# snap-research/InstantRestore

Hardware: AMD Instinct MI355X
Metric: restored images/sec @512px, 4 refs, single-step; 1/2/4/8 MI355X (higher is better)
Workload: dtype bf16

## Files before the change

instantrestore_amd/csrc/linear_tiled.hip:

```cpp
#include <stdlib.h>
#include <type_traits>

#include "ir_common.h"
#include "ir_colstats.h"
#include "ir_kernels.h"

namespace {

constexpr int kTiledPitch = 144;

template <typename T, int WM, int WN, int MI, int NI, bool XF32, bool ILV, int KW = 1>
__global__ void __launch_bounds__(WM * WN * KW * 64, KW == 1 ? 2 : 1) linear_tiled_kernel(const LinearKParams p) {
  using Tr = ElemTraits<T>;
  using v8 = typename Tr::v8;
  using v4 = typename Tr::v4;
  constexpr int NW = WM * WN, NT = NW * 64;
  constexpr int BM = WM * MI * 32, BN = WN * NI * 32;
  constexpr int XT = BM * 128, WT = BN * 128, STAGE = XT + WT;
  constexpr int XP = BM / 8 / NW, WP = BN / 8 / NW;
  constexpr int XU = BM * 8 / NT;
  static_assert(BM % (8 * NW) == 0 && BN % (8 * NW) == 0, "pieces must divide over the waves");
  extern __shared__ __attribute__((aligned(16))) unsigned char dsm_tiled[];
  const int lane = threadIdx.x & 63;
  const int wid_all = __builtin_amdgcn_readfirstlane(threadIdx.x >> 6);
  const int kg = KW == 1 ? 0 : wid_all / NW;
  const int wid = KW == 1 ? wid_all : wid_all - kg * NW;
  const int tid = wid * 64 + lane;
  unsigned char* const smem = dsm_tiled + kg * (2 * STAGE);

  const int wm = wid / WN, wn = wid - wm * WN;
  const int hi = lane >> 5, lq = lane & 31;

  const int MT = (p.M + BM - 1) / BM, NTl = p.N / BN;
  const int logical = xcd_remap((int)blockIdx.x, MT * NTl);
  const int GM = p.nsplit;
  const int grp = logical / (GM * NTl), rem = logical - grp * (GM * NTl);
  const int gm = (MT - grp * GM) < GM ? (MT - grp * GM) : GM;
  const int tm = grp * GM + rem % gm, tn = rem / gm;
  const int m0 = tm * BM, n0 = tn * BN;
  const int rows_valid = (p.M - m0) < BM ? (p.M - m0) : BM;
  const int KT = (p.K >> 6) / KW;
  const int kt0 = kg * KT;

  const T* const wbase = (const T*)p.w + (int64_t)n0 * p.w_ld;
  const i32x4 wrs = make_rsrc_words(wbase, (unsigned)(((int64_t)(BN - 1) * p.w_ld + p.K) * 2));
  unsigned wvo[WP];
#pragma unroll
  for (int j = 0; j < WP; ++j) {
    const int row = 8 * (wid + j * NW) + (lane >> 3);
    wvo[j] = (unsigned)(row * p.w_ld * 2 + ((((lane & 7) ^ ((row >> 1) & 7))) << 4));
  }
  i32x4 xrs = wrs;
  unsigned xvo[XF32 ? 1 : XP];
  const float* xfp[XF32 ? XU : 1];
  int xlds[XF32 ? XU : 1];
  if constexpr (!XF32) {
    const T* const xbase = (const T*)p.x + (int64_t)m0 * p.x_ld;
    xrs = make_rsrc_words(xbase, (unsigned)(((int64_t)(rows_valid - 1) * p.x_ld + p.K) * 2));
#pragma unroll
    for (int j = 0; j < XP; ++j) {
      const int row = 8 * (wid + j * NW) + (lane >> 3);
      xvo[j] = (unsigned)(row * p.x_ld * 2 + ((((lane & 7) ^ ((row >> 1) & 7))) << 4));
    }
  } else {
#pragma unroll
    for (int j = 0; j < XU; ++j) {
      const int u = tid + j * NT, row = u >> 3, ch = u & 7;
      const int gr = (m0 + row) < p.M ? (m0 + row) : (p.M - 1);
      xfp[j] = (const float*)p.x + (int64_t)gr * p.x_ld + ch * 8;
      xlds[j] = row * 128 + ((ch ^ ((row >> 1) & 7)) << 4);
    }
  }
  constexpr int NPIECE = WP + (XF32 ? 0 : XP);
  auto issue_piece = [&](int j, int kt, int slot) {
    unsigned char* const sx = smem + slot * STAGE;
    if (j < WP) buffer_load_lds16_async(wrs, sx + XT + (wid + j * NW) * 1024, wvo[j] + (kt0 + kt) * 128);
    else if constexpr (!XF32) buffer_load_lds16_async(xrs, sx + (wid + (j - WP) * NW) * 1024, xvo[j - WP] + (kt0 + kt) * 128);
  };
  auto issue_dma = [&](int kt, int slot) {
#pragma unroll
    for (int j = 0; j < NPIECE; ++j) issue_piece(j, kt, slot);
  };
  f32x4 xr[XF32 ? XU : 1][2];
  auto load_x32 = [&](int kt) {
    if constexpr (XF32) {
#pragma unroll
      for (int j = 0; j < XU; ++j) {
        asm volatile("global_load_dwordx4 %0, %1, off" : "=v"(xr[j][0]) : "v"(xfp[j] + (kt0 + kt) * 64) : "memory");
        asm volatile("global_load_dwordx4 %0, %1, off offset:16" : "=v"(xr[j][1]) : "v"(xfp[j] + (kt0 + kt) * 64) : "memory");
      }
    }
  };
  auto put_x32 = [&](int slot) {
    if constexpr (XF32) {
      unsigned char* const sx = smem + slot * STAGE;
      asm volatile("s_waitcnt vmcnt(0)" : "+v"(xr[0][0]), "+v"(xr[0][1]) : : "memory");
#pragma unroll
      for (int j = 1; j < XU; ++j) asm volatile("" : "+v"(xr[j][0]), "+v"(xr[j][1]));
#pragma unroll
      for (int j = 0; j < XU; ++j) {
        const f32x8 f = __builtin_shufflevector(xr[j][0], xr[j][1], 0, 1, 2, 3, 4, 5, 6, 7);
        *(IR_LDS v8*)(IR_LDS unsigned char*)(sx + xlds[j]) = __builtin_convertvector(f, v8);
      }
    }
  };

  int fread[4];
#pragma unroll
  for (int ks = 0; ks < 4; ++ks) fread[ks] = lq * 128 + (((2 * ks + hi) ^ ((lq >> 1) & 7)) << 4);
  const int xrow0 = wm * (MI * 32) * 128, wrow0 = XT + wn * (NI * 32) * 128;

  f32x16 acc[MI][NI];
#pragma unroll
  for (int mi = 0; mi < MI; ++mi)
#pragma unroll
    for (int ni = 0; ni < NI; ++ni)
#pragma unroll
      for (int r = 0; r < 16; ++r) acc[mi][ni][r] = 0.f;

  constexpr int HALF_MFMA = 2 * MI * NI;
  constexpr int STRIDE = (HALF_MFMA / NPIECE) > 0 ? (HALF_MFMA / NPIECE) : 1;
  auto compute = [&](int slot, int dma_kt, int dma_slot) {
    const unsigned char* const st = smem + slot * STAGE;
    v8 wf[2][NI], xf[2][MI];
    auto rd = [&](int ks, int b) {
#pragma unroll
      for (int ni = 0; ni < NI; ++ni) wf[b][ni] = *(const IR_LDS v8*)(IR_LDS unsigned char*)(st + wrow0 + ni * 4096 + fread[ks]);
#pragma unroll
      for (int mi = 0; mi < MI; ++mi) xf[b][mi] = *(const IR_LDS v8*)(IR_LDS unsigned char*)(st + xrow0 + mi * 4096 + fread[ks]);
    };
    rd(0, 0);
#pragma unroll
    for (int ks = 0; ks < 4; ++ks) {
      if (ks + 1 < 4) rd(ks + 1, (ks + 1) & 1);
#pragma unroll
      for (int mi = 0; mi < MI; ++mi)
#pragma unroll
        for (int ni = 0; ni < NI; ++ni) {
          acc[mi][ni] = Tr::mfma(wf[ks & 1][ni], xf[ks & 1][mi], acc[mi][ni]);
          if constexpr (ILV) {
            const int m = ks * MI * NI + mi * NI + ni;
            if (m < HALF_MFMA && (m % STRIDE) == STRIDE - 1 && (m / STRIDE) < NPIECE) {
              __builtin_amdgcn_sched_barrier(0);
              if (dma_kt >= 0) issue_piece(m / STRIDE, dma_kt, dma_slot);
              __builtin_amdgcn_sched_barrier(0);
            }
            if (m == HALF_MFMA - 1) {
#pragma unroll
              for (int j = HALF_MFMA / STRIDE; j < NPIECE; ++j)
                if (dma_kt >= 0) issue_piece(j, dma_kt, dma_slot);
            }
          }
        }
    }
  };

  issue_dma(0, 0);
  load_x32(0);
  put_x32(0);
  asm volatile("s_waitcnt vmcnt(0)" ::: "memory");
  __syncthreads();
  for (int kt = 0; kt + 1 < KT; ++kt) {
    const int cur = kt & 1;
    if constexpr (!ILV) issue_dma(kt + 1, cur ^ 1);
    load_x32(kt + 1);
    compute(cur, kt + 1, cur ^ 1);
    put_x32(cur ^ 1);
    asm volatile("s_waitcnt vmcnt(0)" ::: "memory");
    __syncthreads();
  }
  compute((KT - 1) & 1, -1, 0);
  __syncthreads();
  if constexpr (KW == 2) {
    constexpr int HAND_OFF = 2 * STAGE;
    static_assert(2 * STAGE >= NW * MI * 32 * kTiledPitch, "epilogue staging must stay below the hand-over area");
    static_assert(2 * STAGE >= NW * MI * NI * 16 * 64 * 4, "hand-over area");
    unsigned char* const hand = dsm_tiled + HAND_OFF + wid * (MI * NI * 16 * 64 * 4) + lane * 16;
    if (kg == 1) {
#pragma unroll
      for (int mi = 0; mi < MI; ++mi)
#pragma unroll
        for (int ni = 0; ni < NI; ++ni)
#pragma unroll
          for (int g = 0; g < 4; ++g)
            *(f32x4_alias*)(hand + ((mi * NI + ni) * 4 + g) * 1024) = f32x4{acc[mi][ni][4 * g], acc[mi][ni][4 * g + 1], acc[mi][ni][4 * g + 2], acc[mi][ni][4 * g + 3]};
    }
    __syncthreads();
    if (kg == 1) return;
#pragma unroll
    for (int mi = 0; mi < MI; ++mi)
#pragma unroll
      for (int ni = 0; ni < NI; ++ni)
#pragma unroll
        for (int g = 0; g < 4; ++g) {
          const f32x4 o = *(const f32x4_alias*)(hand + ((mi * NI + ni) * 4 + g) * 1024);
#pragma unroll
          for (int i = 0; i < 4; ++i) acc[mi][ni][4 * g + i] += o[i];
        }
  }

  unsigned char* const tb = smem + wid * (MI * 32 * kTiledPitch);
  const int row_base = m0 + wm * (MI * 32);
  v4 bvs[NI][4];
  if (p.bias != nullptr) {
#pragma unroll
    for (int ni = 0; ni < NI; ++ni)
#pragma unroll
      for (int g = 0; g < 4; ++g) bvs[ni][g] = *(const v4*)((const T*)p.bias + n0 + wn * (NI * 32) + ni * 32 + 8 * g + 4 * hi);
  } else {
#pragma unroll
    for (int ni = 0; ni < NI; ++ni)
#pragma unroll
      for (int g = 0; g < 4; ++g) bvs[ni][g] = v4{0, 0, 0, 0};
  }
#pragma unroll
  for (int nh = 0; nh < NI / 2; ++nh) {
    const int ncol0 = n0 + wn * (NI * 32) + nh * 64;
#pragma unroll
    for (int n2 = 0; n2 < 2; ++n2) {
      const int ni = 2 * nh + n2;
      const float cs = (ncol0 + n2 * 32) < p.scale_cols ? p.col_scale : 1.0f;
#pragma unroll
      for (int g = 0; g < 4; ++g) {
        f32x4 bz;
#pragma unroll
        for (int i = 0; i < 4; ++i) bz[i] = (float)bvs[ni][g][i];
#pragma unroll
        for (int mi = 0; mi < MI; ++mi) {
          f32x4 f;
#pragma unroll
          for (int i = 0; i < 4; ++i) f[i] = acc[mi][ni][4 * g + i] * cs + bz[i];
          *(v4*)(tb + (mi * 32 + lq) * kTiledPitch + n2 * 64 + (8 * g + 4 * hi) * 2) = __builtin_convertvector(f, v4);
        }
      }
    }
    ir_wave_lds_fence();
    const int st_head = (ncol0 - p.st_col0) >> 6;
    const bool st_on = p.st_ws != nullptr && ncol0 >= p.st_col0 && st_head < (p.st_cols >> 6) && row_base < p.M;
    ColStatsAcc sacc;
#pragma unroll
    for (int j = 0; j < MI * 4; ++j) {
      const int r = 8 * j + (lane >> 3);
      const u32x4 v = *(const u32x4_alias*)(tb + r * kTiledPitch + (lane & 7) * 16);
      const int row = row_base + r;
      if (row < p.M) ir_store_y((u32x4*)((T*)p.y + (int64_t)row * p.y_ld + ncol0 + (lane & 7) * 8), v);
      if (st_on) {
        if (j == 0) ir_stats_first<T>(sacc, v);
        else ir_stats_add<T>(sacc, v);
      }
    }
    ir_wave_lds_fence();
    if (st_on) ir_stats_finish(sacc, p.st_ws + ((int64_t)(row_base / kStatsRows) * (p.st_cols >> 6) + st_head) * 128);
  }
}


template <typename T, bool XF32>
__global__ void __launch_bounds__(512, 2) linear_tiled_pp_kernel(const LinearKParams p) {
  using Tr = ElemTraits<T>;
  using v8 = typename Tr::v8;
  using v4 = typename Tr::v4;
  constexpr int NW = 8, NT = 512, WN = 2, MI = 2, NI = 4;
  constexpr int BM = 256, BN = 256;
  constexpr int XT = BM * 128, WT = BN * 128, STAGE = XT + WT;
  constexpr int XP = BM / 8 / NW, WP = BN / 8 / NW;
  constexpr int XU = BM * 8 / NT;
  constexpr int OUT_OFF = 2 * STAGE;
  extern __shared__ __attribute__((aligned(16))) unsigned char dsm_tiled_pp[];
  unsigned char* const smem = dsm_tiled_pp;

  const int tid = threadIdx.x;
  const int lane = tid & 63;
  const int wid = __builtin_amdgcn_readfirstlane(tid >> 6);
  const int grp = wid >> 2;
  const int wm = wid / WN, wn = wid - wm * WN;
  const int hi = lane >> 5, lq = lane & 31;
  const int KT = p.K >> 6;

  const int MT = (p.M + BM - 1) / BM, NTl = (p.N + BN - 1) / BN;
  const int ntiles = MT * NTl;
  const int xcd = blockIdx.x & 7, xs = blockIdx.x >> 3;
  const int q8 = ntiles >> 3, r8 = ntiles & 7;
  const int t_start = (xcd < r8) ? xcd * (q8 + 1) : r8 * (q8 + 1) + (xcd - r8) * q8;
  const int t_count = q8 + (xcd < r8 ? 1 : 0);
  const int wg_x = ((int)gridDim.x >> 3) + (xcd < ((int)gridDim.x & 7) ? 1 : 0);

  unsigned wvo[WP], xvo[XF32 ? 1 : XP];
  int xlds0 = 0;
#pragma unroll
  for (int j = 0; j < WP; ++j) {
    const int row = 8 * (wid + j * NW) + (lane >> 3);
    wvo[j] = (unsigned)(row * p.w_ld * 2 + ((((lane & 7) ^ ((row >> 1) & 7))) << 4));
  }
  if constexpr (!XF32) {
#pragma unroll
    for (int j = 0; j < XP; ++j) {
      const int row = 8 * (wid + j * NW) + (lane >> 3);
      xvo[j] = (unsigned)(row * p.x_ld * 2 + ((((lane & 7) ^ ((row >> 1) & 7))) << 4));
    }
  } else {
    const int row = tid >> 3, ch = tid & 7;
    xlds0 = row * 128 + ((ch ^ ((row >> 1) & 7)) << 4);
  }
  int fread[4];
#pragma unroll
  for (int ks = 0; ks < 4; ++ks) fread[ks] = lq * 128 + (((2 * ks + hi) ^ ((lq >> 1) & 7)) << 4);
  const int xrow0 = wm * (MI * 32) * 128, wrow0 = XT + wn * (NI * 32) * 128;

  int m0 = 0, n0 = 0;
  i32x4 wrs = {0, 0, 0, 0}, xrs = {0, 0, 0, 0};
  const float* xtile = nullptr;
  unsigned xoff[XF32 ? XU : 1];
  auto set_tile = [&](int logical) {
    const int GM = p.nsplit;
    const int tgrp = logical / (GM * NTl), rem = logical - tgrp * (GM * NTl);
    const int gm = (MT - tgrp * GM) < GM ? (MT - tgrp * GM) : GM;
    const int tm = tgrp * GM + rem % gm, tn = rem / gm;
    m0 = tm * BM; n0 = tn * BN;
    const int rows_valid = (p.M - m0) < BM ? (p.M - m0) : BM;
    const int cols_valid = (p.N - n0) < BN ? (p.N - n0) : BN;
    wrs = make_rsrc_words((const T*)p.w + (int64_t)n0 * p.w_ld, (unsigned)(((int64_t)(cols_valid - 1) * p.w_ld + p.K) * 2));
    if constexpr (!XF32) {
      xrs = make_rsrc_words((const T*)p.x + (int64_t)m0 * p.x_ld, (unsigned)(((int64_t)(rows_valid - 1) * p.x_ld + p.K) * 2));
    } else {
      xtile = (const float*)p.x + (int64_t)m0 * p.x_ld;
#pragma unroll
      for (int j = 0; j < XU; ++j) {
        const int row = (tid >> 3) + 64 * j;
        const int rr = row < rows_valid ? row : rows_valid - 1;
        xoff[j] = (unsigned)(rr * (int)p.x_ld + (tid & 7) * 8) * 4u;
      }
    }
  };
  f32x4 xr[XF32 ? XU : 1][2];
  auto issue_w = [&](int kt, int slot) {
    unsigned char* const sx = smem + slot * STAGE;
#pragma unroll
    for (int j = 0; j < WP; ++j) buffer_load_lds16_async(wrs, sx + XT + (wid + j * NW) * 1024, wvo[j] + kt * 128);
  };
  auto issue_x = [&](int kt, int slot) {
    if constexpr (!XF32) {
      unsigned char* const sx = smem + slot * STAGE;
#pragma unroll
      for (int j = 0; j < XP; ++j) buffer_load_lds16_async(xrs, sx + (wid + j * NW) * 1024, xvo[j] + kt * 128);
    } else {
#pragma unroll
      for (int j = 0; j < XU; ++j) {
        const unsigned o = xoff[j] + (unsigned)kt * 256u;
        asm volatile("s_nop 4\n\tglobal_load_dwordx4 %0, %1, %2" : "=v"(xr[j][0]) : "v"(o), "s"(xtile) : "memory");
        asm volatile("global_load_dwordx4 %0, %1, %2 offset:16" : "=v"(xr[j][1]) : "v"(o), "s"(xtile) : "memory");
      }
    }
  };
  auto land_stage = [&](int slot) {
    if constexpr (XF32) {
      unsigned char* const sx = smem + slot * STAGE;
      asm volatile("s_waitcnt vmcnt(0)" : "+v"(xr[0][0]), "+v"(xr[0][1]) : : "memory");
#pragma unroll
      for (int j = 1; j < XU; ++j) asm volatile("" : "+v"(xr[j][0]), "+v"(xr[j][1]));
#pragma unroll
      for (int j = 0; j < XU; ++j) {
        const f32x8 f = __builtin_shufflevector(xr[j][0], xr[j][1], 0, 1, 2, 3, 4, 5, 6, 7);
        *(IR_LDS v8*)(IR_LDS unsigned char*)(sx + xlds0 + j * 8192) = __builtin_convertvector(f, v8);
      }
    } else {
      asm volatile("s_waitcnt vmcnt(0)" ::: "memory");
    }
  };

  f32x16 acc[MI][NI];
  v8 wf[2][NI], xf[2][MI];
  auto load_frags = [&](int slot, int half) {
    const unsigned char* const st = smem + slot * STAGE;
#pragma unroll
    for (int q = 0; q < 2; ++q) {
#pragma unroll
      for (int ni = 0; ni < NI; ++ni) wf[q][ni] = *(const IR_LDS v8*)(IR_LDS unsigned char*)(st + wrow0 + ni * 4096 + fread[2 * half + q]);
#pragma unroll
      for (int mi = 0; mi < MI; ++mi) xf[q][mi] = *(const IR_LDS v8*)(IR_LDS unsigned char*)(st + xrow0 + mi * 4096 + fread[2 * half + q]);
    }
  };
  auto matrix_phase = [&]() {
    __builtin_amdgcn_s_setprio(1);
#pragma unroll
    for (int q = 0; q < 2; ++q)
#pragma unroll
      for (int mi = 0; mi < MI; ++mi)
#pragma unroll
        for (int ni = 0; ni < NI; ++ni) acc[mi][ni] = Tr::mfma(wf[q][ni], xf[q][mi], acc[mi][ni]);
    __builtin_amdgcn_s_setprio(0);
  };
  auto phase_end = [&]() {
    __builtin_amdgcn_sched_barrier(0);
    asm volatile("s_waitcnt lgkmcnt(0)" ::: "memory");
    __builtin_amdgcn_s_barrier();
    __builtin_amdgcn_sched_barrier(0);
  };
  auto epilogue = [&](int em0, int en0) {
    unsigned char* const tb = smem + OUT_OFF + wid * 4096;
#pragma unroll
    for (int nh = 0; nh < NI / 2; ++nh) {
      const int ncol0 = en0 + wn * (NI * 32) + nh * 64;
      if (ncol0 >= p.N) break;
      v4 bvs[2][4];
      if (p.bias != nullptr) {
#pragma unroll
        for (int n2 = 0; n2 < 2; ++n2)
#pragma unroll
          for (int g = 0; g < 4; ++g) bvs[n2][g] = *(const v4*)((const T*)p.bias + ncol0 + n2 * 32 + 8 * g + 4 * hi);
      } else {
#pragma unroll
        for (int n2 = 0; n2 < 2; ++n2)
#pragma unroll
          for (int g = 0; g < 4; ++g) bvs[n2][g] = v4{0, 0, 0, 0};
      }
      const int st_head = (ncol0 - p.st_col0) >> 6;
      const bool st_on = p.st_ws != nullptr && ncol0 >= p.st_col0 && st_head < (p.st_cols >> 6) && (em0 + wm * (MI * 32)) < p.M;
      ColStatsAcc sacc;
#pragma unroll
      for (int mi = 0; mi < MI; ++mi) {
#pragma unroll
        for (int half = 0; half < 2; ++half) {
          if ((lq >> 4) == half) {
#pragma unroll
            for (int n2 = 0; n2 < 2; ++n2) {
              const float cs = (ncol0 + n2 * 32) < p.scale_cols ? p.col_scale : 1.0f;
#pragma unroll
              for (int g = 0; g < 4; ++g) {
                f32x4 f;
#pragma unroll
                for (int i = 0; i < 4; ++i) f[i] = acc[mi][2 * nh + n2][4 * g + i] * cs + (float)bvs[n2][g][i];
                *(v4*)(tb + (lq & 15) * kTiledPitch + n2 * 64 + (8 * g + 4 * hi) * 2) = __builtin_convertvector(f, v4);
              }
            }
          }
          ir_wave_lds_fence();
#pragma unroll
          for (int j = 0; j < 2; ++j) {
            const int r = 8 * j + (lane >> 3);
            const u32x4 v = *(const u32x4_alias*)(tb + r * kTiledPitch + (lane & 7) * 16);
            const int row = em0 + wm * (MI * 32) + mi * 32 + half * 16 + r;
            if (row < p.M) ir_store_y((u32x4*)((T*)p.y + (int64_t)row * p.y_ld + ncol0 + (lane & 7) * 8), v);
            if (st_on) {
              if (mi == 0 && half == 0 && j == 0) ir_stats_first<T>(sacc, v);
              else ir_stats_add<T>(sacc, v);
            }
          }
          ir_wave_lds_fence();
        }
      }
      if (st_on) ir_stats_finish(sacc, p.st_ws + ((int64_t)((em0 + wm * (MI * 32)) / kStatsRows) * (p.st_cols >> 6) + st_head) * 128);
    }
  };

  if (xs >= t_count) return;
  set_tile(t_start + xs);
  issue_w(0, 0);
  issue_x(0, 0);
  for (int tl = xs; tl < t_count; tl += wg_x) {
#pragma unroll
    for (int mi = 0; mi < MI; ++mi)
#pragma unroll
      for (int ni = 0; ni < NI; ++ni)
#pragma unroll
        for (int r = 0; r < 16; ++r) acc[mi][ni][r] = 0.f;
    land_stage(0);
    asm volatile("s_waitcnt vmcnt(0)" ::: "memory");
    phase_end();
    load_frags(0, 0);
    if (KT > 1) { issue_w(1, 1); issue_x(1, 1); }
    if (grp == 1) phase_end();
    for (int kt = 0; kt < KT; ++kt) {
      const int cur = kt & 1;
      matrix_phase();
      phase_end();
      load_frags(cur, 1);
      if (kt + 1 < KT) land_stage(cur ^ 1);
      phase_end();
      matrix_phase();
      phase_end();
      if (kt + 1 < KT) {
        load_frags(cur ^ 1, 0);
        if (kt + 2 < KT) { issue_w(kt + 2, cur); issue_x(kt + 2, cur); }
      }
      phase_end();
    }
    if (grp == 0) phase_end();
    const int em0 = m0, en0 = n0;
    const bool more = tl + wg_x < t_count;
    if (more) {
      set_tile(t_start + tl + wg_x);
      issue_w(0, 0);
      if constexpr (!XF32) issue_x(0, 0);
    }
    epilogue(em0, en0);
    if constexpr (XF32) { if (more) issue_x(0, 0); }
  }
}


static int walk_group_rows() {
  static const int gm = [] { const char* e = getenv("IR_LIN_GM"); const int v = e ? atoi(e) : 0; return (v >= 1 && v <= 64) ? v : 4; }();
  return gm;
}

template <typename T, bool XF32>
hipError_t launch_pp(const LinearKParams& p0, hipStream_t s) {
  LinearKParams p = p0;
  p.nsplit = walk_group_rows();
  constexpr size_t dyn = 2 * (size_t)(256 + 256) * 128 + 8 * 4096;
  static IrOncePerDevice once;
  static std::atomic<int> n_cu[64];
  int dev = -1;
  const hipError_t ea = ir_opt_in_dynamic_lds(once, (const void*)linear_tiled_pp_kernel<T, XF32>, dyn, &dev);
  if (ea != hipSuccess) return ea;
  int cus = (dev >= 0 && dev < 64) ? n_cu[dev].load(std::memory_order_relaxed) : 0;
  if (cus <= 0) {
    if (hipDeviceGetAttribute(&cus, hipDeviceAttributeMultiprocessorCount, dev < 0 ? 0 : dev) != hipSuccess || cus <= 0) cus = 256;
    if (dev >= 0 && dev < 64) n_cu[dev].store(cus, std::memory_order_relaxed);
  }
  const int MT = (p.M + 255) / 256, NTl = (p.N + 255) / 256;
  const int ntiles = MT * NTl;
  static const bool persistent = [] { const char* e = getenv("IR_LIN_PERSISTENT"); return e == nullptr || e[0] != '0'; }();
  const int grid = (persistent && ntiles > cus) ? cus : ntiles;
  hipLaunchKernelGGL((linear_tiled_pp_kernel<T, XF32>), dim3((unsigned)grid), dim3(512), dyn, s, p);
  return hipGetLastError();
}

template <typename T, int WM, int WN, int MI, int NI, bool XF32, bool ILV, int KW = 1>
hipError_t launch_cfg(const LinearKParams& p0, hipStream_t s) {
  LinearKParams p = p0;
  p.nsplit = walk_group_rows();
  constexpr int BM = WM * MI * 32, BN = WN * NI * 32;
  constexpr size_t stage = (size_t)(BM + BN) * 128;
  constexpr size_t epi = (size_t)WM * WN * MI * 32 * kTiledPitch;
  constexpr size_t dyn = KW * 2 * stage > epi ? KW * 2 * stage : epi;
  if (KW == 2 && ((p.K >> 6) & 1)) return hipErrorInvalidValue;
  static IrOncePerDevice once;
  const hipError_t ea = ir_opt_in_dynamic_lds(once, (const void*)linear_tiled_kernel<T, WM, WN, MI, NI, XF32, ILV, KW>, dyn);
  if (ea != hipSuccess) return ea;
  const int MT = (p.M + BM - 1) / BM, NTl = p.N / BN;
  hipLaunchKernelGGL((linear_tiled_kernel<T, WM, WN, MI, NI, XF32, ILV, KW>), dim3((unsigned)(MT * NTl)), dim3(WM * WN * KW * 64), dyn, s, p);
  return hipGetLastError();
}

template <typename T, bool XF32>
hipError_t launch_x(const LinearKParams& p, int cfg, hipStream_t s) {
  constexpr bool I = true;
  switch (cfg) {
    case IR_LIN_TILE_256x128: return launch_cfg<T, 4, 2, 2, 2, XF32, I>(p, s);
    case IR_LIN_TILE_128x128: return launch_cfg<T, 2, 2, 2, 2, XF32, I>(p, s);
    case IR_LIN_TILE_128x64: return launch_cfg<T, 2, 1, 2, 2, XF32, I>(p, s);
    case IR_LIN_TILE_256x64: return launch_cfg<T, 4, 1, 2, 2, XF32, I>(p, s);
    case IR_LIN_TILE_64x128: return launch_cfg<T, 1, 2, 2, 2, XF32, I>(p, s);
    case IR_LIN_TILE_128x256: return launch_cfg<T, 2, 2, 2, 4, XF32, I>(p, s);
    case IR_LIN_TILE_128x128_K2: return launch_cfg<T, 2, 2, 2, 2, XF32, I, 2>(p, s);
    case IR_LIN_TILE_256x256: return launch_pp<T, XF32>(p, s);
    default: return hipErrorInvalidValue;
  }
}

}

int ir_linear_tiled_pick(int64_t M, int N, int K) {
  auto tiles = [&](int bm, int bn) { return ((M + bm - 1) / bm) * (int64_t)((N + bn - 1) / bn); };
  if (tiles(256, 256) >= 160) return IR_LIN_TILE_256x256;
  if (N % 128 == 0 && tiles(128, 128) >= 128 && tiles(128, 128) <= 256 && K >= 1024 && ((K >> 6) & 1) == 0) return IR_LIN_TILE_128x128_K2;
  if (N % 128 == 0) return tiles(128, 128) >= 128 ? IR_LIN_TILE_128x128 : IR_LIN_TILE_64x128;
  return tiles(256, 64) >= 512 ? IR_LIN_TILE_256x64 : IR_LIN_TILE_128x64;
}

bool ir_linear_tiled_cfg_ok(int cfg, int N) {
  switch (cfg) {
    case IR_LIN_TILE_256x128: case IR_LIN_TILE_128x128: case IR_LIN_TILE_64x128: case IR_LIN_TILE_128x128_K2: return N % 128 == 0;
    case IR_LIN_TILE_128x64: case IR_LIN_TILE_256x64: return N % 64 == 0;
    case IR_LIN_TILE_128x256: return N % 256 == 0;
    case IR_LIN_TILE_256x256: return N % 64 == 0;
    default: return false;
  }
}

hipError_t ir_launch_linear_tiled(const LinearKParams& p, int dtype, int cfg, hipStream_t s) {
  if (dtype == 1) return p.x_f32 ? launch_x<__bf16, true>(p, cfg, s) : launch_x<__bf16, false>(p, cfg, s);
  return p.x_f32 ? launch_x<_Float16, true>(p, cfg, s) : launch_x<_Float16, false>(p, cfg, s);
}
```

Measured before the change: 1226.

## Rework pingpong GEMM epilogue with swizzled staging in stage-1 LDS

The epilogue now stages output tiles in the second pipeline stage's LDS region using an XOR swizzle instead of a padded dedicated buffer. It writes all rows of a 64-column slab before one fence and one batch of reads, replacing per-half write/fence/read cycles. Bias loads are hoisted out of the column loop. The extra 32KB of dynamic LDS is removed, and the next tile's X prefetch is issued before the epilogue for the XF32 case too. It also drops an explicit vmcnt wait after landing stage 0. Reusing the stage-1 region risks a race with the prefetch of the next tile, which lands in stage 0, and with any stage-1 data still in flight.

```diff
diff --git a/instantrestore_amd/csrc/linear_tiled.hip b/instantrestore_amd/csrc/linear_tiled.hip
--- a/instantrestore_amd/csrc/linear_tiled.hip
+++ b/instantrestore_amd/csrc/linear_tiled.hip
@@ -265,7 +265,6 @@
   constexpr int XT = BM * 128, WT = BN * 128, STAGE = XT + WT;
   constexpr int XP = BM / 8 / NW, WP = BN / 8 / NW;
   constexpr int XU = BM * 8 / NT;
-  constexpr int OUT_OFF = 2 * STAGE;
   extern __shared__ __attribute__((aligned(16))) unsigned char dsm_tiled_pp[];
   unsigned char* const smem = dsm_tiled_pp;
 
@@ -397,59 +396,67 @@
     __builtin_amdgcn_sched_barrier(0);
   };
   auto epilogue = [&](int em0, int en0) {
-    unsigned char* const tb = smem + OUT_OFF + wid * 4096;
+    unsigned char* const tb = smem + STAGE + wid * 8192;
+    int el = (int)__builtin_amdgcn_mbcnt_hi(~0u, __builtin_amdgcn_mbcnt_lo(~0u, 0u));
+    asm volatile("" : "+v"(el));
+    const int ehi = el >> 5, elq = el & 31;
+    const int row_base = em0 + wm * (MI * 32);
+    v4 bvs[NI / 2][2][4];
+#pragma unroll
+    for (int nh = 0; nh < NI / 2; ++nh) {
+      const int ncol0 = en0 + wn * (NI * 32) + nh * 64;
+      if (p.bias != nullptr && ncol0 < p.N) {
+#pragma unroll
+        for (int n2 = 0; n2 < 2; ++n2)
+#pragma unroll
+          for (int g = 0; g < 4; ++g) bvs[nh][n2][g] = *(const v4*)((const T*)p.bias + ncol0 + n2 * 32 + 8 * g + 4 * ehi);
+#pragma unroll
+        for (int n2 = 0; n2 < 2; ++n2)
+#pragma unroll
+          for (int g = 0; g < 4; ++g) asm volatile("" : "+v"(bvs[nh][n2][g]));
+      } else {
+#pragma unroll
+        for (int n2 = 0; n2 < 2; ++n2)
+#pragma unroll
+          for (int g = 0; g < 4; ++g) bvs[nh][n2][g] = v4{0, 0, 0, 0};
+      }
+    }
 #pragma unroll
     for (int nh = 0; nh < NI / 2; ++nh) {
       const int ncol0 = en0 + wn * (NI * 32) + nh * 64;
       if (ncol0 >= p.N) break;
-      v4 bvs[2][4];
-      if (p.bias != nullptr) {
-#pragma unroll
-        for (int n2 = 0; n2 < 2; ++n2)
-#pragma unroll
-          for (int g = 0; g < 4; ++g) bvs[n2][g] = *(const v4*)((const T*)p.bias + ncol0 + n2 * 32 + 8 * g + 4 * hi);
-      } else {
-#pragma unroll
-        for (int n2 = 0; n2 < 2; ++n2)
-#pragma unroll
-          for (int g = 0; g < 4; ++g) bvs[n2][g] = v4{0, 0, 0, 0};
-      }
       const int st_head = (ncol0 - p.st_col0) >> 6;
-      const bool st_on = p.st_ws != nullptr && ncol0 >= p.st_col0 && st_head < (p.st_cols >> 6) && (em0 + wm * (MI * 32)) < p.M;
+      const bool st_on = p.st_ws != nullptr && ncol0 >= p.st_col0 && st_head < (p.st_cols >> 6) && row_base < p.M;
       ColStatsAcc sacc;
 #pragma unroll
-      for (int mi = 0; mi < MI; ++mi) {
-#pragma unroll
-        for (int half = 0; half < 2; ++half) {
-          if ((lq >> 4) == half) {
-#pragma unroll
-            for (int n2 = 0; n2 < 2; ++n2) {
-              const float cs = (ncol0 + n2 * 32) < p.scale_cols ? p.col_scale : 1.0f;
-#pragma unroll
-              for (int g = 0; g < 4; ++g) {
-                f32x4 f;
-#pragma unroll
-                for (int i = 0; i < 4; ++i) f[i] = acc[mi][2 * nh + n2][4 * g + i] * cs + (float)bvs[n2][g][i];
-                *(v4*)(tb + (lq & 15) * kTiledPitch + n2 * 64 + (8 * g + 4 * hi) * 2) = __builtin_convertvector(f, v4);
-              }
-            }
+      for (int mi = 0; mi < MI; ++mi)
+#pragma unroll
+        for (int n2 = 0; n2 < 2; ++n2) {
+          const float cs = (ncol0 + n2 * 32) < p.scale_cols ? p.col_scale : 1.0f;
+#pragma unroll
+          for (int g = 0; g < 4; ++g) {
+            f32x4 f;
+#pragma unroll
+            for (int i = 0; i < 4; ++i) f[i] = acc[mi][2 * nh + n2][4 * g + i] * cs + (float)bvs[nh][n2][g][i];
+            *(v4*)(tb + (mi * 32 + elq) * 128 + (((n2 * 4 + g) ^ (elq & 7)) << 4) + ehi * 8) = __builtin_convertvector(f, v4);
           }
-          ir_wave_lds_fence();
-#pragma unroll
-          for (int j = 0; j < 2; ++j) {
-            const int r = 8 * j + (lane >> 3);
-            const u32x4 v = *(const u32x4_alias*)(tb + r * kTiledPitch + (lane & 7) * 16);
-            const int row = em0 + wm * (MI * 32) + mi * 32 + half * 16 + r;
-            if (row < p.M) ir_store_y((u32x4*)((T*)p.y + (int64_t)row * p.y_ld + ncol0 + (lane & 7) * 8), v);
-            if (st_on) {
-              if (mi == 0 && half == 0 && j == 0) ir_stats_first<T>(sacc, v);
-              else ir_stats_add<T>(sacc, v);
-            }
-          }
-          ir_wave_lds_fence();
         }
-      }
-      if (st_on) ir_stats_finish(sacc, p.st_ws + ((int64_t)((em0 + wm * (MI * 32)) / kStatsRows) * (p.st_cols >> 6) + st_head) * 128);
+      ir_wave_lds_fence();
+      u32x4 v[MI * 4];
+#pragma unroll
+      for (int j = 0; j < MI * 4; ++j)
+        v[j] = *(const u32x4_alias*)(tb + (8 * j + (el >> 3)) * 128 + (((el & 7) ^ (el >> 3)) << 4));
+      ir_wave_lds_fence();
+#pragma unroll
+      for (int j = 0; j < MI * 4; ++j) {
+        const int row = row_base + 8 * j + (el >> 3);
+        if (row < p.M) ir_store_y((u32x4*)((T*)p.y + (int64_t)row * p.y_ld + ncol0 + (el & 7) * 8), v[j]);
+        if (st_on) {
+          if (j == 0) ir_stats_first<T>(sacc, v[j]);
+          else ir_stats_add<T>(sacc, v[j]);
+        }
+      }
+      if (st_on) ir_stats_finish(sacc, p.st_ws + ((int64_t)(row_base / kStatsRows) * (p.st_cols >> 6) + st_head) * 128);
     }
   };
 
@@ -465,7 +472,6 @@
 #pragma unroll
         for (int r = 0; r < 16; ++r) acc[mi][ni][r] = 0.f;
     land_stage(0);
-    asm volatile("s_waitcnt vmcnt(0)" ::: "memory");
     phase_end();
     load_frags(0, 0);
     if (KT > 1) { issue_w(1, 1); issue_x(1, 1); }
@@ -491,10 +497,9 @@
     if (more) {
       set_tile(t_start + tl + wg_x);
       issue_w(0, 0);
-      if constexpr (!XF32) issue_x(0, 0);
+      issue_x(0, 0);
     }
     epilogue(em0, en0);
-    if constexpr (XF32) { if (more) issue_x(0, 0); }
   }
 }
 
@@ -508,7 +513,7 @@
 hipError_t launch_pp(const LinearKParams& p0, hipStream_t s) {
   LinearKParams p = p0;
   p.nsplit = walk_group_rows();
-  constexpr size_t dyn = 2 * (size_t)(256 + 256) * 128 + 8 * 4096;
+  constexpr size_t dyn = 2 * (size_t)(256 + 256) * 128;
   static IrOncePerDevice once;
   static std::atomic<int> n_cu[64];
   int dev = -1;
```

Result: no change. 1224, median of 3 (-0.1%).
